# jai1215snu/ShiftedScaleQuantization

Hardware: AMD Instinct MI355X
Metric: Gelem/s shifted-scale q/dq + recon iters/s, ResNet-18 W2A4; top-1 vs ref (higher is better)
Workload: dtype f32; 1 GPU; resnet18 W2A4 bias_cal+bias_ch_quant, 1024 calib samples: A4 per-tensor q/dq of act [1024,64,56,56] + W2 per-channel q/dq of all 21 conv/fc weights (8-bit stem/head); parallelism=dp1

## Files before the change

include/ssq.h:

```cpp
#ifndef SSQ_H_
#define SSQ_H_

#include <stddef.h>
#include <stdint.h>

#ifdef __cplusplus
extern "C" {
#endif

#define SSQ_OK 0
#define SSQ_E_ARG (-1)
#define SSQ_E_WS (-2)

typedef void* ssq_stream_t;

const char* ssq_last_error(void);
int ssq_version(void);
int ssq_set_variant(int variant);

int ssq_fq_fwd(const float* x, float* y, void* codes_or_null, const float* delta,
               const float* zp, int64_t n, int64_t inner, int64_t nch, float scale,
               int qmin, int qmax, ssq_stream_t stream);
int ssq_fq_round_fwd(const float* x, float* y, void* codes_or_null, const float* delta,
                     const float* zp, int64_t n, int64_t inner, int64_t nch, float scale,
// ... 170 lines not shown
int ssq_epilogue_bwd(const float* g, const float* y, const float* bias, const float* gamma,
                     const float* phi, const float* res, int64_t N, int64_t C, int64_t hw,
                     int relu, const float* delta, const float* zp, int qmin, int qmax, float* gy,
                     float* gres, float* ggamma, float* gphi, float* gdelta, float* gzp, void* ws,
                     size_t ws_bytes, ssq_stream_t stream);
int ssq_epilogue_loss_bwd(const float* tgt_cache, const int64_t* idx, int64_t M, float p,
                          float* loss_out, const float* y, const float* bias, const float* gamma,
                          const float* phi, const float* res, const float* res_bias,
                          const float* res_gamma, const float* res_phi, int64_t N, int64_t C,
                          int64_t hw, int relu, const float* delta, const float* zp, int qmin,
                          int qmax, float* gy, float* gres, float* ggamma, float* gphi,
                          float* gres_gamma, float* gres_phi, float* gdelta, float* gzp,
                          void* ws, size_t ws_bytes, ssq_stream_t stream);
int ssq_epilogue_fwd_rows(const float* y, const int64_t* y_rows, const float* bias,
                          const float* gamma, const float* phi, const float* res,
                          const int64_t* res_rows, float* out, float* yq, int64_t n, int64_t hw,
                          int64_t C, int relu, const float* delta, const float* zp, int qmin,
                          int qmax, const int64_t* stage_src, int64_t* stage_dst,
                          int64_t stage_n, ssq_stream_t stream);
int ssq_epilogue_bwd_rows(const float* g, const float* y, const int64_t* y_rows,
                          const float* bias, const float* gamma, const float* phi,
                          const float* res, const int64_t* res_rows, int64_t N, int64_t C,
                          int64_t hw, int relu, const float* delta, const float* zp, int qmin,
                          int qmax, float* gy, float* gres, float* ggamma, float* gphi,
                          float* gdelta, float* gzp, void* ws, size_t ws_bytes,
                          ssq_stream_t stream);
int ssq_epilogue_loss_bwd_rows(const float* tgt_cache, const int64_t* idx, int64_t M, float p,
                               float* loss_out, const float* y, const int64_t* y_rows,
                               const float* bias, const float* gamma, const float* phi,
                               const float* res, const int64_t* res_rows,
                               const float* res_bias, const float* res_gamma,
                               const float* res_phi, int64_t N, int64_t C, int64_t hw, int relu,
                               const float* delta, const float* zp, int qmin, int qmax,
                               float* gy, float* gres, float* ggamma, float* gphi,
                               float* gres_gamma, float* gres_phi, float* gdelta, float* gzp,
                               void* ws, size_t ws_bytes, ssq_stream_t stream);

int ssq_adam(int nseg, float* const* p, const float* const* g, float* const* m,
             float* const* v, const int64_t* n, float one_minus_beta1, float beta2,
             float one_minus_beta2, float eps, const float* hyper, float neg_step_size,
             float bias_correction2_sqrt, ssq_stream_t stream);
int ssq_adam_arm(int nseg, float* const* p, float* const* m, float* const* v, const int64_t* n,
                 float one_minus_beta1, float beta2, float one_minus_beta2, float eps,
                 const float* hyper, ssq_stream_t stream);
int ssq_adam_take(ssq_stream_t stream);

int ssq_set_deferred_finalize(int on);
int ssq_flush_finalize(ssq_stream_t stream);

int ssq_set_deferred_prep_fwd(int on);
int ssq_flush_prep_fwd(ssq_stream_t stream);

int ssq_conv_wgrad_set_form(int form);
int ssq_conv_wgrad_kind(int64_t Nb, int64_t C, int64_t H, int64_t W, int64_t Co, int64_t R,
                        int64_t S, int64_t stride, int64_t pad, int64_t groups);
size_t ssq_conv_wgrad_workspace_size(int64_t Nb, int64_t C, int64_t H, int64_t W, int64_t Co,
                                     int64_t R, int64_t S, int64_t stride, int64_t pad,
                                     int64_t groups);
int ssq_conv_wgrad(const float* x, const float* dy, int64_t Nb, int64_t C, int64_t H, int64_t W,
                   int64_t Co, int64_t R, int64_t S, int64_t stride, int64_t pad, int64_t groups,
                   float* dw, void* ws, size_t ws_bytes, ssq_stream_t stream);
int ssq_wgrad_gemm_operands(const float* x, const float* dy, int64_t Nb, int64_t C, int64_t H,
                            int64_t W, int64_t Co, int64_t R, int64_t S, int64_t stride,
                            int64_t pad, float* col, float* dy2, ssq_stream_t stream);
int ssq_gemm_col_epilogue(const float* y, const float* bias, const float* gamma,
                          const float* phi, int relu, const float* delta, const float* zp,
                          int qmin, int qmax, int64_t Nb, int64_t C, int64_t H, int64_t W,
                          int64_t R, int64_t S, int64_t stride, int64_t pad, float* col,
                          ssq_stream_t stream);

int ssq_dwconv_supported(int64_t Nb, int64_t C, int64_t H, int64_t W, int64_t R, int64_t S,
                         int64_t stride, int64_t pad);
int ssq_dwconv_fwd(const float* x, const float* w, float* y, int64_t Nb, int64_t C, int64_t H,
                   int64_t W, int64_t R, int64_t S, int64_t stride, int64_t pad,
                   ssq_stream_t stream);
int ssq_dwconv_bwd_data(const float* dy, const float* w, float* dx, int64_t Nb, int64_t C,
                        int64_t H, int64_t W, int64_t R, int64_t S, int64_t stride, int64_t pad,
                        ssq_stream_t stream);

int ssq_pack_bits(int n_bits);
size_t ssq_pack_bytes(int64_t n, int n_bits);
int ssq_pack_encode(const float* What, const float* zp, const float* d1, int d1_per_ci,
                    const float* d2, int64_t Co, int64_t Ci, int64_t K, int n_bits, int qmin,
                    int qmax, void* packed, uint32_t* mismatch, ssq_stream_t stream);
int ssq_pack_decode(const void* packed, const float* zp, const float* d1, int d1_per_ci,
                    const float* d2, int64_t Co, int64_t Ci, int64_t K, int n_bits, int qmin,
                    float* What, ssq_stream_t stream);

int ssq_stream_copy(const float* src, float* dst, int64_t n, ssq_stream_t stream);
int ssq_stream_probe(const float* src, float* dst, int64_t n, int kind, ssq_stream_t stream);

#ifdef __cplusplus
}
#endif
#endif
```

shiftedscalequantization_amd/_capi.py:

```python
import ctypes as C
import os

import torch

_HERE = os.path.dirname(os.path.abspath(__file__))
LIB_PATH = os.environ.get("SSQ_LIB", os.path.join(_HERE, "libssq.so"))

_p = C.c_void_p
_i64 = C.c_int64
_i = C.c_int
_f = C.c_float
_sz = C.c_size_t

SIGNATURES = {
    "ssq_last_error": (C.c_char_p, []),
    "ssq_version": (_i, []),
    "ssq_set_variant": (_i, [_i]),
    "ssq_fq_fwd": (_i, [_p, _p, _p, _p, _p, _i64, _i64, _i64, _f, _i, _i, _p]),
    "ssq_fq_round_fwd": (_i, [_p, _p, _p, _p, _p, _i64, _i64, _i64, _f, _i, _i, _p]),
    "ssq_fq_fwd_multi": (_i, [_i, _p, _p, _p, _p, _p, _p, _p, _p, _p, _p]),
    "ssq_fq_bwd_workspace_size": (_sz, [_i64, _i64, _i64]),
    "ssq_fq_bwd": (_i, [_p, _p, _p, _p, _i64, _i64, _i64, _i, _i, _p, _p, _p, _p, _sz, _p]),
    "ssq_fq_round_bwd": (_i, [_p, _p, _p, _p, _i64, _i64, _i64, _i, _i, _p, _p, _p, _sz, _p]),
    "ssq_fq_relu_bwd": (_i, [_p, _p, _p, _p, _i64, _i, _i, _p, _p, _p, _p, _sz, _p]),
# ... 22 lines not shown
                              _f, _f, _p, _p, _p, _p, _p, _sz, _p]),
    "ssq_shift_reg": (_i, [_p, _i, _i64, _i, _f, _f, _p, _p, _p]),
    "ssq_lhs_fwd": (_i, [_p, _p, _p, _p, _p, _i, _i64, _i64, _i64, _i, _i, _i, _i, _p, _p]),
    "ssq_lhs_bwd": (_i, [_p, _p, _p, _p, _p, _p, _i, _i64, _i64, _i64, _i, _i, _i, _p, _p, _sz,
                         _p]),
    "ssq_adaround_fwd": (_i, [_p, _p, _p, _i, _p, _f, _i64, _i64, _i64, _i, _i, _i, _p, _p, _p]),
    "ssq_adaround_bwd": (_i, [_p, _p, _p, _p, _i, _p, _f, _i64, _i64, _i64, _i, _i, _f, _f, _p,
                              _p, _p]),
    "ssq_adaround_fwd_multi": (_i, [_i, _p, _p, _p, _p, _p, _p, _p, _p, _p, _i, _p, _p, _p, _p]),
    "ssq_adaround_bwd_multi": (_i, [_i, _p, _p, _p, _p, _p, _p, _p, _p, _p, _p, _p, _p, _f, _f,
                                    _p, _p, _p]),
    "ssq_round_reg_workspace_size": (_sz, [_i64]),
    "ssq_round_reg": (_i, [_p, _i64, _f, _f, _p, _p, _p, _sz, _p]),
    "ssq_inpscale_search": (_i, [_p, _p, _p, _i64, _i64, _i, _i, _f, _p, _p]),
    "ssq_inpscale_fwd": (_i, [_p, _p, _p, _p, _i64, _i64, _i, _p, _p]),
    "ssq_lp_loss_workspace_size": (_sz, [_i64]),
    "ssq_lp_loss": (_i, [_p, _p, _i64, _i64, _f, _p, _p, _p, _i, _p, _sz, _p]),
    "ssq_lp_loss_rows": (_i, [_p, _p, _p, _i64, _i64, _i64, _f, _p, _p, _p, _i, _p, _sz, _p]),
    "ssq_gather_rows2": (_i, [_p, _p, _i64, _p, _p, _i64, _p, _i64, _p]),
    "ssq_gemm_col_epilogue": (_i, [_p, _p, _p, _p, _i, _p, _p, _i, _i] + [_i64] * 8 + [_p, _p]),
    "ssq_fc_recon_workspace_size": (_sz, [_i64, _i64, _i64]),
    "ssq_fc_recon_iter": (_i, [_p, _p, _p, _i64, _p, _p, _p, _p, _p, _i, _i, _p, _i64, _i64, _f, _f,
                               _f, _f, _p, _p, _p, _p, _p, _p, _sz, _p]),
    "ssq_gather_rows2_staged": (_i, [_p, _p, _i64, _p, _p, _i64, _p, _i64, _p, _i64, _p]),
    "ssq_bias_act": (_i, [_p, _p, _p, _p, _i64, _i64, _i64, _i, _p]),
    "ssq_relu_bwd": (_i, [_p, _p, _p, _i64, _p]),
    "ssq_relu6_bwd": (_i, [_p, _p, _p, _i64, _p]),
    "ssq_bias_act_fq": (_i, [_p, _p, _p, _p, _p, _i64, _i64, _i64, _i, _p, _p, _i, _i, _p]),
    "ssq_epilogue_fwd": (_i, [_p, _p, _p, _p, _p, _p, _p, _i64, _i64, _i64, _i, _p, _p, _i, _i,
                              _p]),
    "ssq_epilogue_bwd_workspace_size": (_sz, [_i64]),
    "ssq_epilogue_bwd": (_i, [_p, _p, _p, _p, _p, _p, _i64, _i64, _i64, _i, _p, _p, _i, _i, _p,
                              _p, _p, _p, _p, _p, _p, _sz, _p]),
    "ssq_epilogue_loss_bwd": (_i, [_p, _p, _i64, _f, _p, _p, _p, _p, _p, _p, _p, _p, _p, _i64,
                                   _i64, _i64, _i, _p, _p, _i, _i, _p, _p, _p, _p, _p, _p, _p,
                                   _p, _p, _sz, _p]),
    "ssq_epilogue_fwd_rows": (_i, [_p, _p, _p, _p, _p, _p, _p, _p, _p, _i64, _i64, _i64, _i, _p,
                                   _p, _i, _i, _p, _p, _i64, _p]),
    "ssq_epilogue_bwd_rows": (_i, [_p, _p, _p, _p, _p, _p, _p, _p, _i64, _i64, _i64, _i, _p, _p,
                                   _i, _i, _p, _p, _p, _p, _p, _p, _p, _sz, _p]),
    "ssq_epilogue_loss_bwd_rows": (_i, [_p, _p, _i64, _f, _p, _p, _p, _p, _p, _p, _p, _p, _p, _p,
                                        _p, _i64, _i64, _i64, _i, _p, _p, _i, _i, _p, _p, _p, _p,
                                        _p, _p, _p, _p, _p, _sz, _p]),
    "ssq_adam": (_i, [_i, _p, _p, _p, _p, _p, _f, _f, _f, _f, _p, _f, _f, _p]),
    "ssq_adam_arm": (_i, [_i, _p, _p, _p, _p, _f, _f, _f, _f, _p, _p]),
    "ssq_adam_take": (_i, [_p]),
    "ssq_set_deferred_finalize": (_i, [_i]),
    "ssq_flush_finalize": (_i, [_p]),
    "ssq_set_deferred_prep_fwd": (_i, [_i]),
    "ssq_set_deferred_fq_multi": (_i, [_i]),
    "ssq_flush_fq_multi": (_i, [_p]),
    "ssq_flush_prep_fwd": (_i, [_p]),
    "ssq_conv_wgrad_set_form": (_i, [_i]),
    "ssq_conv_wgrad_kind": (_i, [_i64] * 10),
    "ssq_conv_wgrad_workspace_size": (_sz, [_i64] * 10),
    "ssq_conv_wgrad": (_i, [_p, _p] + [_i64] * 10 + [_p, _p, _sz, _p]),
    "ssq_wgrad_gemm_operands": (_i, [_p, _p] + [_i64] * 9 + [_p, _p, _p]),
    "ssq_maxpool2d_fwd": (_i, [_p, _p] + [_i64] * 7 + [_p]),
    "ssq_dwconv_supported": (_i, [_i64] * 8),
    "ssq_dwconv_fwd": (_i, [_p, _p, _p] + [_i64] * 8 + [_p]),
    "ssq_dwconv_bwd_data": (_i, [_p, _p, _p] + [_i64] * 8 + [_p]),
    "ssq_pack_bits": (_i, [_i]),
    "ssq_pack_bytes": (_sz, [_i64, _i]),
    "ssq_pack_encode": (_i, [_p, _p, _p, _i, _p, _i64, _i64, _i64, _i, _i, _i, _p, _p, _p]),
    "ssq_pack_decode": (_i, [_p, _p, _p, _i, _p, _i64, _i64, _i64, _i, _i, _p, _p]),
    "ssq_stream_copy": (_i, [_p, _p, _i64, _p]),
    "ssq_stream_probe": (_i, [_p, _p, _i64, _i, _p]),
}

_lib = None


class SSQError(RuntimeError):
    pass


def load():
    global _lib
    if _lib is not None:
        return _lib
    if not os.path.exists(LIB_PATH):
        raise SSQError(f"libssq.so not found at {LIB_PATH}; build it with "
                       "`python -m shiftedscalequantization_amd.build` (hipcc, gfx950)")
    lib = C.CDLL(LIB_PATH)
    for name, (res, args) in SIGNATURES.items():
        fn = getattr(lib, name)
        fn.restype = res
        fn.argtypes = args
    _lib = lib
    return lib


CALL_HOOK = None


def call(name, *args):
    lib = load()
    if CALL_HOOK is not None:
        CALL_HOOK(name, args)
    rc = getattr(lib, name)(*args)
    if rc != 0:
        msg = lib.ssq_last_error().decode(errors="replace")
        raise SSQError(f"{name} failed (rc={rc}): {msg}")


def query(name, *args):
# ... 95 lines not shown
```

shiftedscalequantization_amd/csrc/conv_wgrad.hip:

```cpp
#include <stdlib.h>

#include <algorithm>
#include <type_traits>

#include "ssq_common.h"

namespace ssq {

typedef float f32x16 __attribute__((ext_vector_type(16)));

constexpr int kUnr = 2;

struct WgradGeo {
  int Nb, C, H, W, Co, OH, OW, R, S, st, pad, G, Cig, Cog;
  int Ncol;
  int WM;
  int Pq;
  int lda;
  int chunks_per_n;
  int nchunks;
  int cps;
  int nsplit;
  int in_rows;
  int ci_span;
// ... 668 lines not shown
    const char* v = getenv("SSQ_K17_MAXLDS");
    return (int64_t)(v && *v ? atoll(v) : 160 * 1024);
  }();
  double best = 1e300;
  for (int wm : {1, 2, 4}) {
    for (int pq : {128, 64}) {
      const int TM = 64 * wm, TN = 256 / wm;
      const int64_t span = std::min<int64_t>(g.Cig, (TN - 1) / RS + 2);
      const int64_t orows = (pq - 1 + OW - 1) / OW + 1;
      const int64_t in_rows = (orows - 1) * st + R;
      const int64_t xtile = span * in_rows * Wp;
      if ((int64_t)wgrad_lds(wm, pq, xtile) > max_lds) continue;
      const int64_t cpn = (OH * OW + pq - 1) / pq;
      const int64_t tiles = ((g.Cog + TM - 1) / TM) * ((g.Ncol + TN - 1) / TN);
      const double dma = (double)(std::min<int64_t>(TM, g.Cog) * ((pq + 63) / 64) +
                                  span * in_rows * ((W + 63) / 64)) / 4.0;
      const double cost = (double)tiles * Nb * (2.0 * OH * OW + cpn * (40.0 + dma));
      if (cost < best) {
        best = cost;
        g.WM = wm;
        g.Pq = pq;
        g.ci_span = (int)span;
        g.in_rows = (int)in_rows;
        g.xtile = (int)xtile;
      }
    }
  }
  SSQ_REQUIRE(best < 1e300, SSQ_E_ARG, "ssq_conv_wgrad: input rows too wide for the LDS tile");
  const int TM = 64 * g.WM, TN = 256 / g.WM;
  g.lda = g.Pq + 1;
  g.chunks_per_n = (int)((OH * OW + g.Pq - 1) / g.Pq);
  g.nchunks = g.Nb * g.chunks_per_n;
  g.m_tiles = (g.Cog + TM - 1) / TM;
  g.n_tiles = (g.Ncol + TN - 1) / TN;
  const int64_t tiles = (int64_t)g.n_tiles * g.m_tiles * g.G;
  int nsplit = (int)std::max<int64_t>(1, std::min<int64_t>(g.nchunks / 2, (512 + tiles - 1) / tiles));
  g.cps = (g.nchunks + nsplit - 1) / nsplit;
  g.nsplit = (g.nchunks + g.cps - 1) / g.cps;
  *lds_bytes = wgrad_lds(g.WM, g.Pq, g.xtile);
  return SSQ_OK;
}

constexpr int kBandMaxNI = 20;
__device__ float g_band_zero_page[4 * 64];

struct BandGeo {
  int C, H, W, Co, OW, OHW, Cig, Cog;
  int RB, Q, Qp, PA, IR, PXrow, PXci;
  int TMc, CBc;
  int bufsz;
  int d16;
  int ni_w;
  int bands_per_n, nchunks, cps, nsplit, m_tiles, n_tiles, remap;
  FastDiv dPA, dPXci, dPXrow;
};

template <int N>
using IntC = std::integral_constant<int, N>;

template <int WMX, int ST, int V, int NWV>
__global__ __launch_bounds__(64 * NWV, 1) void wgrad_band_stage1(const float* __restrict__ x,
                                                                 const float* __restrict__ dy,
                                                                 BandGeo g, float* __restrict__ part) {
  static_assert(NWV == 4 || NWV == 8, "4 or 8 waves");
  constexpr int WNX = 4 / WMX;
  constexpr int kSlots = kBandMaxNI * 4 / NWV;
  extern __shared__ float lds[];
  const int tid = threadIdx.x, lane = tid & 63;
  const int wave = __builtin_amdgcn_readfirstlane(tid >> 6);
  const int wt = wave & 3, role = wave >> 2;
  const int wm = wt / WNX, wn = wt - wm * WNX;
  int wg = blockIdx.x;
  const int tiles = g.m_tiles * g.n_tiles;
  if (g.remap) {
    const int per = (int)gridDim.x >> 3;
    wg = (wg & 7) * per + (wg >> 3);
  }
  const int split = wg / tiles, tile = wg - split * tiles;
  const int mt = tile / g.n_tiles, nt = tile - mt * g.n_tiles;
  const int co0 = mt * g.TMc, ci0 = nt * g.CBc;
  const int c_begin = split * g.cps, c_end = min(c_begin + g.cps, g.nchunks);
  const int abytes = g.TMc * g.PA;
  const int n16 = g.d16 ? min(kSlots, (g.bufsz / 256 - wave + NWV - 1) / NWV) : 0;
  const int n4 = g.d16 ? 0 : (g.bufsz / 64 - wave + NWV - 1) / NWV;

  int soff[kSlots], meta[kSlots];
#pragma unroll
  for (int i = 0; i < kSlots; ++i) {
    soff[i] = 0;
    meta[i] = 0;
    if (i < n16) {
      const int o = (wave + NWV * i) * 256 + lane * 4;
      if (o < abytes) {
        const int row = (int)fdiv((uint32_t)o, g.dPA), col = o - row * g.PA;
        if (col < g.Q && co0 + row < g.Cog) {
          soff[i] = (co0 + row) * g.OHW + col;
          meta[i] = 1;
        }
      } else {
        const int o2 = o - abytes;
        const int cl = (int)fdiv((uint32_t)o2, g.dPXci), rem = o2 - cl * g.PXci;
        const int ir = (int)fdiv((uint32_t)rem, g.dPXrow), iw = rem - ir * g.PXrow - 4;
        if (cl < g.CBc && ci0 + cl < g.Cig && ir < g.IR && iw >= 0 && iw < g.W) {
          soff[i] = ((ci0 + cl) * g.H + ir) * g.W + iw;
          meta[i] = 2 | (ir << 2);
        }
      }
    }
  }
  struct Band {
    const float* ab;
    const float* xb;
    int ih0;
  };
  auto band_of = [&](int c) {
    const int n = c / g.bands_per_n;
    const int oh0 = (c - n * g.bands_per_n) * g.RB;
    const int ih0 = oh0 * ST - 1;
    return Band{dy + (int64_t)n * g.Co * g.OHW + oh0 * g.OW,
                x + (int64_t)n * g.C * g.H * g.W + (int64_t)ih0 * g.W, ih0};
  };
  auto stage16 = [&](const Band& bd, int b) {
    const float* zero = g_band_zero_page + lane * 4;
    float* dst = lds + b * g.bufsz + wave * 256;
#pragma unroll
    for (int i = 0; i < kSlots; ++i) {
      if (i < n16) {
        const int kind = meta[i] & 3;
        const unsigned ih = (unsigned)(bd.ih0 + (meta[i] >> 2));
        const bool ok = (kind == 1) | ((kind == 2) & (ih < (unsigned)g.H));
        const uint64_t pa = (uint64_t)(bd.ab + soff[i]), px = (uint64_t)(bd.xb + soff[i]);
        const uint64_t p = ok ? (kind == 1 ? pa : px) : (uint64_t)zero;
        __builtin_amdgcn_global_load_lds((const void*)p, (void*)(dst + i * NWV * 256), 16, 0, 0);
      }
    }
  };
  const int HW = g.H * g.W;
  auto stage4 = [&](const Band& bd, int b, int i0, int i1) {
    const float* zero = g_band_zero_page + lane;
    float* dst = lds + b * g.bufsz + wave * 64;
    for (int i = i0; i < i1; ++i) {
      const int o = (wave + NWV * i) * 64 + lane;
      const float* src = zero;
      if ((wave + NWV * i) * 64 < abytes) {
        const int row = (int)fdiv((uint32_t)o, g.dPA), col = o - row * g.PA;
        if (col < g.Q && co0 + row < g.Cog) src = bd.ab + (co0 + row) * g.OHW + col;
      } else {
        const int o2 = o - abytes;
        const int cl = (int)fdiv((uint32_t)o2, g.dPXci), rem = o2 - cl * g.PXci;
        const int ir = (int)fdiv((uint32_t)rem, g.dPXrow), iw = rem - ir * g.PXrow - 4;
        const unsigned ih = (unsigned)(bd.ih0 + ir);
        if (cl < g.CBc && ci0 + cl < g.Cig && ir < g.IR && iw >= 0 && iw < g.W &&
            ih < (unsigned)g.H)
          src = bd.xb + (ci0 + cl) * HW + ir * g.W + iw;
      }
      __builtin_amdgcn_global_load_lds((const void*)src, (void*)(dst + i * NWV * 64), 4, 0, 0);
    }
  };

  typedef float f32x4v __attribute__((ext_vector_type(4)));
  typedef float f32x2v __attribute__((ext_vector_type(2)));
  const int h = lane >> 5, l32 = lane & 31;
  const int arow = (wm * 32 + l32) * g.PA;
  const int xrow = abytes + (wn * 32 + l32) * g.PXci;
  const int q0 = h * (g.Qp >> 1);
  const int ngroups = g.Qp / (2 * V);
  const int last_row = (g.Q - 1) / g.OW, last_col = (g.Q - 1) - last_row * g.OW;
  constexpr int NW = (V - 1) * ST + 3;
  const int per_step = (n4 + max(1, ngroups / 2) - 1) / max(1, ngroups / 2);
  if (c_begin < c_end) {
    const Band bd = band_of(c_begin);
    if (g.d16) stage16(bd, 0);
    else stage4(bd, 0, 0, n4);
  }

  auto body = [&](auto t0c, auto t1c) {
    constexpr int T0 = decltype(t0c)::value, T1 = decltype(t1c)::value, NT = T1 - T0;
    constexpr int R0 = T0 / 3, NR = (T1 - 1) / 3 - R0 + 1;
    f32x16 acc[NT];
#pragma unroll
    for (int t = 0; t < NT; ++t) acc[t] = f32x16{0};
    auto fetch = [&](const float* L, int q, int orow, int ow, float (&a)[V],
                     float (&w)[NR][NW]) {
      if constexpr (V == 4) {
        const f32x4v av = *(const f32x4v*)(L + arow + q);
        a[0] = av.x; a[1] = av.y; a[2] = av.z; a[3] = av.w;
      } else if constexpr (V == 2) {
        const f32x2v av = *(const f32x2v*)(L + arow + q);
        a[0] = av.x; a[1] = av.y;
      } else {
        a[0] = L[arow + q];
      }
      int xr_row = orow, xr_col = ow;
      if (q >= g.Q) {
        xr_row = last_row;
        xr_col = last_col - (V - 1);
      }
      const float* xr0 = L + xrow + (xr_row * ST + R0) * g.PXrow + xr_col * ST + 3;
#pragma unroll
      for (int r = 0; r < NR; ++r) {
        const float* xr = xr0 + r * g.PXrow;
        if constexpr (V == 4) {
          w[r][0] = xr[0];
          const f32x4v t1 = *(const f32x4v*)(xr + 1);
          w[r][1] = t1.x; w[r][2] = t1.y; w[r][3] = t1.z; w[r][4] = t1.w;
          if constexpr (ST == 1) {
            w[r][5] = xr[5];
          } else {
            const f32x4v t2 = *(const f32x4v*)(xr + 5);
            w[r][5] = t2.x; w[r][6] = t2.y; w[r][7] = t2.z; w[r][8] = t2.w;
          }
        } else {
#pragma unroll
          for (int j = 0; j < NW; ++j) w[r][j] = xr[j];
        }
      }
    };
    auto mfmas = [&](const float (&a)[V], const float (&w)[NR][NW]) {
#pragma unroll
      for (int r = 0; r < NR; ++r)
#pragma unroll
        for (int v = 0; v < V; ++v)
#pragma unroll
          for (int s = 0; s < 3; ++s) {
            const int tap = (R0 + r) * 3 + s;
            if (tap >= T0 && tap < T1)
              acc[tap - T0] = __builtin_amdgcn_mfma_f32_32x32x2f32(a[v], w[r][v * ST + s],
                                                                   acc[tap - T0], 0, 0, 0);
          }
    };
    auto interleave = [&]() {
      constexpr int NM = NT * V, ND = NM < 12 ? NM : 12;
#pragma unroll
      for (int k = 0; k < ND; ++k) {
        __builtin_amdgcn_sched_group_barrier(0x008, 1, 0);
        __builtin_amdgcn_sched_group_barrier(0x100, 1, 0);
      }
      __builtin_amdgcn_sched_group_barrier(0x008, NM - ND, 0);
    };
    for (int c = c_begin; c < c_end; ++c) {
      const int b = (c - c_begin) & 1;
      asm volatile("s_waitcnt vmcnt(0)" ::: "memory");
      __syncthreads();
      const bool more = c + 1 < c_end;
      const Band nb = band_of(more ? c + 1 : c);
      if (more && g.d16) stage16(nb, b ^ 1);
      const float* L = lds + b * g.bufsz;
      int q = q0, orow = q0 / g.OW, ow = q0 - orow * g.OW;
      auto advance = [&]() {
        q += V;
        ow += V;
        if (ow == g.OW) {
          ow = 0;
          ++orow;
        }
      };
      auto stage_slice = [&](int gi) {
        if (more && !g.d16) {
          const int i0 = gi * per_step;
          if (i0 < n4) stage4(nb, b ^ 1, i0, min(i0 + per_step, n4));
        }
      };
      float a0[V], w0[NR][NW], a1[V], w1[NR][NW];
      fetch(L, q, orow, ow, a0, w0);
      const int npairs = ngroups >> 1;
      for (int gp = 0; gp < npairs; ++gp) {
        stage_slice(2 * gp);
        advance();
        fetch(L, q, orow, ow, a1, w1);
        mfmas(a0, w0);
        interleave();
        stage_slice(2 * gp + 1);
        advance();
        fetch(L, q, orow, ow, a0, w0);
        mfmas(a1, w1);
        interleave();
      }
      if (ngroups & 1) {
        stage_slice(ngroups - 1);
        mfmas(a0, w0);
      }
    }
    const int co_w = co0 + wm * 32, ci = ci0 + wn * 32 + l32;
    if (ci < g.Cig) {
#pragma unroll
      for (int t = 0; t < NT; ++t) {
        float* dst = part + ((int64_t)split * 9 + T0 + t) * g.Cog * g.Cig;
#pragma unroll
        for (int i = 0; i < 16; ++i) {
          const int co = co_w + (i & 3) + 8 * (i >> 2) + 4 * h;
          if (co < g.Cog) dst[(int64_t)co * g.Cig + ci] = acc[t][i];
        }
      }
    }
  };
  if constexpr (NWV == 4) {
    body(IntC<0>{}, IntC<9>{});
  } else {
    if (role == 0) body(IntC<0>{}, IntC<5>{});
    else body(IntC<5>{}, IntC<9>{});
  }
}

static int g_wgrad_form = 0;
static int band_waves() {
  static const int w = [] {
    const char* e = getenv("SSQ_BAND_WAVES");
    return e && *e && atoi(e) == 4 ? 4 : 8;
  }();
  return g_wgrad_form == 4 ? 4 : w;
}

static int band_plan(int64_t Nb, int64_t C, int64_t H, int64_t W, int64_t Co, int64_t R,
                     int64_t S, int64_t st, int64_t pad, int64_t G, BandGeo& g, int* wmx,
                     int* vpx) {
  if (G != 1 || R != 3 || S != 3 || pad != 1 || (st != 1 && st != 2)) return 0;
  const int64_t OH = (H + 2 - 3) / st + 1, OW = (W + 2 - 3) / st + 1;
  if (OH < 1 || OW < 1 || Co % 32 || C % 32) return 0;
  if (Nb * C * H * W >= (1ll << 31) || Nb * Co * OH * OW >= (1ll << 31)) return 0;
  g.C = (int)C; g.H = (int)H; g.W = (int)W; g.Co = (int)Co; g.OW = (int)OW;
  g.OHW = (int)(OH * OW); g.Cig = (int)C; g.Cog = (int)Co;
  const int V = OW % 4 == 0 ? 4 : (OW % 2 == 0 ? 2 : 1);
  auto odd4 = [](int v) { v = (v + 3) / 4 * 4; return (v / 4) % 2 ? v : v + 4; };
  const int64_t budget = 160 * 1024 / 2 / 4;
  bool found = false;
  double best = 1e300;
  for (int wm : {2, 4}) {
    const int TMc = 32 * wm, CBc = 32 * (4 / wm);
    if (wm == 4 && Co < 128) continue;
    for (int rb = (int)std::min<int64_t>(OH, 8); rb >= 1; --rb) {
      if (OH % rb) continue;
      const int Q = rb * (int)OW, Qp = (Q + 2 * V - 1) / (2 * V) * (2 * V);
      const int IR = (rb - 1) * (int)st + 3;
      const bool d16 = W % 4 == 0 && g.OHW % 4 == 0 && Q % 4 == 0 && Qp == Q;
      const int need = (int)((OW - 1) * st) + 6;
      const int PXrow = d16 ? (int)W + 8 : (std::max<int>(need, (int)W + 4) + 3) / 4 * 4;
      const int PA = odd4(Qp + 1), PXci = odd4(IR * PXrow);
      const int64_t buf = ((int64_t)TMc * PA + (int64_t)CBc * PXci + 1023) / 1024 * 1024;
      if (buf > budget) continue;
      const int ni = d16 ? (int)(buf / 1024) : (int)(buf / 256);
      if (d16 && ni > kBandMaxNI) continue;
      const double cost = (288.0 * Qp + 1500.0 + (d16 ? 40.0 : 10.0) * ni) / Q;
      if (cost >= best) continue;
      best = cost;
      g.RB = rb; g.Q = Q; g.Qp = Qp; g.PA = PA; g.IR = IR; g.PXrow = PXrow; g.PXci = PXci;
      g.TMc = TMc; g.CBc = CBc; g.bufsz = (int)buf; g.d16 = d16 ? 1 : 0; g.ni_w = ni;
      *wmx = wm;
      *vpx = V;
      found = true;
    }
  }
  if (!found) return 0;
  g.dPA = make_fastdiv((uint32_t)g.PA);
  g.dPXci = make_fastdiv((uint32_t)g.PXci);
  g.dPXrow = make_fastdiv((uint32_t)g.PXrow);
  g.m_tiles = (g.Cog + g.TMc - 1) / g.TMc;
  g.n_tiles = (g.Cig + g.CBc - 1) / g.CBc;
  g.bands_per_n = (int)(OH / g.RB);
  g.nchunks = (int)Nb * g.bands_per_n;
  const int tiles = g.m_tiles * g.n_tiles;
  int ns = std::max(1, std::min(g.nchunks, (256 + tiles - 1) / tiles));
  g.cps = (g.nchunks + ns - 1) / ns;
  g.nsplit = (g.nchunks + g.cps - 1) / g.cps;
  g.remap = ((int64_t)g.nsplit * tiles) % 8 == 0;
  return 1;
}

static bool use_band(int64_t Nb, int64_t C, int64_t H, int64_t W, int64_t Co, int64_t R,
                     int64_t S, int64_t st, int64_t pad, int64_t G, BandGeo& g, int* wmx,
                     int* vpx) {
  if (g_wgrad_form != 0 && g_wgrad_form != 3 && g_wgrad_form != 4) return false;
  return band_plan(Nb, C, H, W, Co, R, S, st, pad, G, g, wmx, vpx) != 0;
}
static bool use_i2c(int64_t R, int64_t S, int64_t Co, int64_t G) {
  if (g_wgrad_form != 0) return g_wgrad_form == 2;
  return R * S > 1 && G == 1 && Co >= 128;
}

}

using namespace ssq;

extern "C" int ssq_conv_wgrad_set_form(int form) {
  const int old = g_wgrad_form;
  if (form >= 0 && form <= 4) g_wgrad_form = form;
  return old;
}

extern "C" int ssq_conv_wgrad_kind(int64_t Nb, int64_t C, int64_t H, int64_t W, int64_t Co,
                                   int64_t R, int64_t S, int64_t stride, int64_t pad,
                                   int64_t groups) {
  if (is_depthwise(C, Co, groups) && R * S <= 25 && Nb >= 1 && dw_lds_ok(H, W, pad)) return 5;
  BandGeo gb;
  int wmx, vpx;
  if (use_band(Nb, C, H, W, Co, R, S, stride, pad, groups, gb, &wmx, &vpx)) return gb.d16 ? 3 : 6;
  if (use_i2c(R, S, Co, groups)) {
    I2cGeo gi;
    return wgrad_i2c_plan(Nb, C, H, W, Co, R, S, stride, pad, groups, gi) ? 0 : 2;
  }
  if (R == 1 && S == 1 && pad == 0) {
    W1Geo g1;
    return wgrad_1x1_plan(Nb, C, H, W, Co, stride, groups, g1) ? 0 : 4;
  }
  WgradGeo g;
  size_t lds;
  return wgrad_plan(Nb, C, H, W, Co, R, S, stride, pad, groups, g, &lds) ? 0 : 1;
}

extern "C" size_t ssq_conv_wgrad_workspace_size(int64_t Nb, int64_t C, int64_t H, int64_t W,
                                                int64_t Co, int64_t R, int64_t S, int64_t stride,
                                                int64_t pad, int64_t groups) {
  if (is_depthwise(C, Co, groups) && R * S <= 25 && Nb >= 1 && dw_lds_ok(H, W, pad)) {
    int spl;
    const int ns = dw_splits(Nb, C, &spl);
    const int64_t OH = (H + 2 * pad - R) / stride + 1;
    int64_t nbands = 1;
    if (dw_stage(H, W, pad, spl) == 0 && OH >= 1) {
      const int bh = dw_band_rows(H, W, R, stride, pad, OH);
      nbands = (OH + bh - 1) / bh;
    }
    return (size_t)ns * (size_t)nbands * (size_t)C * (size_t)(R * S) * sizeof(float);
  }
  {
    BandGeo gb;
    int wmx, vpx;
    if (use_band(Nb, C, H, W, Co, R, S, stride, pad, groups, gb, &wmx, &vpx))
      return (size_t)gb.nsplit * 9 * (size_t)Co * (size_t)C * sizeof(float);
  }
  if (use_i2c(R, S, Co, groups)) {
    I2cGeo gi;
    int wm;
    if (wgrad_i2c_plan(Nb, C, H, W, Co, R, S, stride, pad, groups, gi)) return 0;
    wgrad_i2c_tiles(gi, &wm);
    return (size_t)gi.nsplit * (size_t)Co * (size_t)gi.Ncol * sizeof(float);
  }
  if (R == 1 && S == 1 && pad == 0) {
    W1Geo g1;
    if (wgrad_1x1_plan(Nb, C, H, W, Co, stride, groups, g1)) return 0;
    return (size_t)g1.nsplit * (size_t)Co * (size_t)g1.Cig * sizeof(float);
// ... 34 lines not shown
      else
        hipLaunchKernelGGL(wgrad_dw_small<25>, grid, dim3(256), lds, s, x, dy, (int)C, (int)H,
                           (int)W, (int)OH, (int)OW, (int)R, (int)S, (int)stride, (int)pad, spl,
                           nb, dWp, dP, dOHW, dOW, (float*)ws);
      const int64_t n = C * R * S;
      hipLaunchKernelGGL(wgrad_stage2, dim3((unsigned)std::min<int64_t>((n + 63) / 64, 4096)),
                         dim3(256), 0, s, (const float*)ws, ns, n, dw);
      return check_launch("ssq_conv_wgrad");
    }
    const int bh = dw_band_rows(H, W, R, stride, pad, OH);
    const int nbands = (int)((OH + bh - 1) / bh);
    SSQ_REQUIRE(ws_bytes >= need * (size_t)nbands, SSQ_E_WS, "ssq_conv_wgrad: workspace too small");
    const dim3 gridb((unsigned)C, (unsigned)(ns * nbands));
    const size_t lds = (size_t)(((int64_t)bh - 1) * stride + R) * (W + 2 * pad) * sizeof(float);
    static bool dw_attr = false;
    if (!dw_attr) {
      hipFuncSetAttribute((const void*)wgrad_dw_stage1<9>,
                          hipFuncAttributeMaxDynamicSharedMemorySize, 128 * 1024);
      hipFuncSetAttribute((const void*)wgrad_dw_stage1<25>,
                          hipFuncAttributeMaxDynamicSharedMemorySize, 128 * 1024);
      dw_attr = true;
    }
    if (R * S <= 9)
      hipLaunchKernelGGL(wgrad_dw_stage1<9>, gridb, dim3(256), lds, s, x, dy, (int)C, (int)H, (int)W,
                         (int)OH, (int)OW, (int)R, (int)S, (int)stride, (int)pad, spl, bh, nbands,
                         make_fastdiv((uint32_t)(W + 2 * pad)), (float*)ws);
    else
      hipLaunchKernelGGL(wgrad_dw_stage1<25>, gridb, dim3(256), lds, s, x, dy, (int)C, (int)H, (int)W,
                         (int)OH, (int)OW, (int)R, (int)S, (int)stride, (int)pad, spl, bh, nbands,
                         make_fastdiv((uint32_t)(W + 2 * pad)), (float*)ws);
    const int64_t n = C * R * S;
    hipLaunchKernelGGL(wgrad_stage2, dim3((unsigned)std::min<int64_t>((n + 63) / 64, 4096)),
                       dim3(256), 0, s, (const float*)ws, ns * nbands, n, dw);
    return check_launch("ssq_conv_wgrad");
  }
  {
    BandGeo gb;
    int wmx, vpx;
    if (use_band(Nb, C, H, W, Co, R, S, stride, pad, groups, gb, &wmx, &vpx)) {
      const size_t needb = (size_t)gb.nsplit * 9 * (size_t)Co * (size_t)C * sizeof(float);
      SSQ_REQUIRE(ws && ws_bytes >= needb, SSQ_E_WS, "ssq_conv_wgrad: workspace too small");
      typedef void (*BandK)(const float*, const float*, BandGeo, float*);
#define SSQ_BK(NWV)                                                                          \
  {{{wgrad_band_stage1<2, 1, 4, NWV>, wgrad_band_stage1<2, 1, 2, NWV>,                        \
     wgrad_band_stage1<2, 1, 1, NWV>},                                                        \
    {wgrad_band_stage1<2, 2, 4, NWV>, wgrad_band_stage1<2, 2, 2, NWV>,                        \
     wgrad_band_stage1<2, 2, 1, NWV>}},                                                       \
   {{wgrad_band_stage1<4, 1, 4, NWV>, wgrad_band_stage1<4, 1, 2, NWV>,                        \
     wgrad_band_stage1<4, 1, 1, NWV>},                                                        \
    {wgrad_band_stage1<4, 2, 4, NWV>, wgrad_band_stage1<4, 2, 2, NWV>,                        \
     wgrad_band_stage1<4, 2, 1, NWV>}}}
      static const BandK kernels[2][2][2][3] = {SSQ_BK(4), SSQ_BK(8)};
#undef SSQ_BK
      static bool band_attr = false;
      if (!band_attr) {
        for (auto& a0 : kernels)
          for (auto& a : a0)
            for (auto& b : a)
              for (BandK k : b)
                hipFuncSetAttribute((const void*)k, hipFuncAttributeMaxDynamicSharedMemorySize,
                                    160 * 1024);
        band_attr = true;
      }
      const int w8 = band_waves() == 8;
      const BandK kb = kernels[w8][wmx == 4][stride == 2][vpx == 4 ? 0 : (vpx == 2 ? 1 : 2)];
      const dim3 gridb((unsigned)(gb.nsplit * gb.m_tiles * gb.n_tiles));
      const size_t ldsb = 2 * (size_t)gb.bufsz * sizeof(float);
      hipLaunchKernelGGL(kb, gridb, dim3(w8 ? 512 : 256), ldsb, s, x, dy, gb, (float*)ws);
      const int64_t inner = Co * C, nb = 9 * inner;
      hipLaunchKernelGGL(wgrad_stage2, dim3((unsigned)std::min<int64_t>((nb + 63) / 64, 4096)),
                         dim3(256), 0, s, (const float*)ws, gb.nsplit, nb, dw, inner, 9);
      return check_launch("ssq_conv_wgrad");
    }
  }
  if (use_i2c(R, S, Co, groups)) {
    I2cGeo gi;
    int wm;
    const int rci = wgrad_i2c_plan(Nb, C, H, W, Co, R, S, stride, pad, groups, gi);
    if (rci) return rci;
    wgrad_i2c_tiles(gi, &wm);
    const size_t needi = (size_t)gi.nsplit * (size_t)Co * (size_t)gi.Ncol * sizeof(float);
    SSQ_REQUIRE(ws && ws_bytes >= needi, SSQ_E_WS, "ssq_conv_wgrad: workspace too small");
    const dim3 gridi(gi.n_tiles, gi.m_tiles * gi.G, gi.nsplit);
    (void)wm;
    hipLaunchKernelGGL(wgrad_i2c_stage1<2>, gridi, dim3(256), 0, s, x, dy, gi, (float*)ws);
    const int64_t ni = (int64_t)Co * gi.Ncol;
    hipLaunchKernelGGL(wgrad_stage2, dim3((unsigned)std::min<int64_t>((ni + 63) / 64, 4096)),
                       dim3(256), 0, s, (const float*)ws, gi.nsplit, ni, dw);
    return check_launch("ssq_conv_wgrad");
  }
  if (R == 1 && S == 1 && pad == 0) {
    W1Geo g1;
    const int rc1 = wgrad_1x1_plan(Nb, C, H, W, Co, stride, groups, g1);
    if (rc1) return rc1;
    const size_t need1 = (size_t)g1.nsplit * (size_t)Co * (size_t)g1.Cig * sizeof(float);
    SSQ_REQUIRE(ws && ws_bytes >= need1, SSQ_E_WS, "ssq_conv_wgrad: workspace too small");
    const dim3 grid1(g1.n_tiles, g1.m_tiles * g1.G, g1.nsplit);
    hipLaunchKernelGGL(wgrad_1x1_stage1<2>, grid1, dim3(256), 0, s, x, dy, g1, (float*)ws);
    const int64_t n1 = (int64_t)Co * g1.Cig;
    hipLaunchKernelGGL(wgrad_stage2, dim3((unsigned)std::min<int64_t>((n1 + 63) / 64, 4096)),
                       dim3(256), 0, s, (const float*)ws, g1.nsplit, n1, dw);
    return check_launch("ssq_conv_wgrad");
  }
  WgradGeo g;
  size_t lds;
  int rc = wgrad_plan(Nb, C, H, W, Co, R, S, stride, pad, groups, g, &lds);
  if (rc) return rc;
  const size_t need = (size_t)g.nsplit * (size_t)Co * (size_t)g.Ncol * sizeof(float);
  SSQ_REQUIRE(ws && ws_bytes >= need, SSQ_E_WS, "ssq_conv_wgrad: workspace too small");
  static bool lds_attr = false;
  if (!lds_attr) {
    hipFuncSetAttribute((const void*)wgrad_stage1<1>, hipFuncAttributeMaxDynamicSharedMemorySize,
                        160 * 1024);
    hipFuncSetAttribute((const void*)wgrad_stage1<2>, hipFuncAttributeMaxDynamicSharedMemorySize,
                        160 * 1024);
    hipFuncSetAttribute((const void*)wgrad_stage1<4>, hipFuncAttributeMaxDynamicSharedMemorySize,
                        160 * 1024);
    lds_attr = true;
  }
  const dim3 grid(g.n_tiles, g.m_tiles * g.G, g.nsplit);
// ... 171 lines not shown
```

shiftedscalequantization_amd/kernels.py:

```python
import ctypes as C
import os

import torch

from . import _capi as A
from ._capi import call, fptr, query, stream_of, workspace


def qrange(n_bits, sym):
    n = 2 ** n_bits
    return (-(n // 2), n // 2 - 1) if sym else (0, n - 1)


def geometry(w):
    if w.dim() == 4:
        return int(w.shape[0]), int(w.shape[1]), int(w.shape[2] * w.shape[3]), 0
    if w.dim() == 2:
        return int(w.shape[0]), int(w.shape[1]), 1, 1
    raise ValueError(f"weight must be 2-D (Linear) or 4-D (Conv2d), got {tuple(w.shape)}")


def _codes_buf(x, want):
    return torch.empty(x.shape, dtype=torch.uint8, device=x.device) if want else None

# ... 1411 lines not shown
    packed = torch.empty(max(nbytes, 1), dtype=torch.uint8, device=w.device)[:nbytes]
    bad = torch.zeros(1, dtype=torch.int32, device=w.device)
    call("ssq_pack_encode", wp, zpp, ap, int(per_ci), bp, Co, Ci, Kk, n_bits, qmin, qmax,
         _vp(packed), _vp(bad), stream_of(w))
    return packed, int(bad.item())


def pack_decode(packed, shape, zp, d1, per_ci, d2, n_bits, qmin):
    if packed.device.type != "cuda" or packed.dtype != torch.uint8:
        raise A.SSQError("pack_decode: packed codes must be a uint8 tensor on the HIP device")
    out = torch.empty(shape, dtype=torch.float32, device=packed.device)
    Co, Ci, Kk, _ = geometry(out)
    if packed.numel() < query("ssq_pack_bytes", out.numel(), n_bits):
        raise A.SSQError("pack_decode: packed buffer too small for the shape")
    packed = packed.contiguous()
    z, zpp = fptr(zp.reshape(-1), "zero_point")
    a, ap = fptr(d1.reshape(-1), "scale")
    b, bp = fptr(d2.reshape(-1), "col_scale") if d2 is not None else (None, None)
    call("ssq_pack_decode", _vp(packed), zpp, ap, int(per_ci), bp, Co, Ci, Kk, n_bits, qmin,
         _vp(out), stream_of(out))
    return out


def conv_wgrad_supported(x, weight, stride, padding, dilation, groups):
    if x.dim() != 4 or weight.dim() != 4 or not x.is_cuda or x.dtype != torch.float32:
        return False
    st = stride if isinstance(stride, int) else stride[0]
    pad = padding if isinstance(padding, int) else padding[0]
    if not isinstance(stride, int) and len(set(stride)) != 1:
        return False
    if not isinstance(padding, int) and (isinstance(padding, str) or len(set(padding)) != 1):
        return False
    if (dilation if isinstance(dilation, int) else max(dilation)) != 1:
        return False
    Nb, C, H, W = (int(v) for v in x.shape)
    Co, _, R, S = (int(v) for v in weight.shape)
    return query("ssq_conv_wgrad_workspace_size", Nb, C, H, W, Co, R, S, int(st), int(pad),
                 int(groups)) > 0


def wgrad_kind(x_shape, w_shape, stride, padding, groups):
    st = stride if isinstance(stride, int) else stride[0]
    pad = padding if isinstance(padding, int) else padding[0]
    Nb, C, H, W = (int(v) for v in x_shape)
    Co, _, R, S = (int(v) for v in w_shape)
    return int(query("ssq_conv_wgrad_kind", Nb, C, H, W, Co, R, S, int(st), int(pad),
                     int(groups)))


def set_wgrad_form(form):
    return int(query("ssq_conv_wgrad_set_form", int(form)))


def conv_wgrad(x, dy, w_shape, stride, padding, groups):
    st = stride if isinstance(stride, int) else stride[0]
    pad = padding if isinstance(padding, int) else padding[0]
    x, xp = fptr(x.detach(), "x")
    dy, dp = fptr(dy.detach(), "dy")
    Nb, C, H, W = (int(v) for v in x.shape)
    Co, _, R, S = (int(v) for v in w_shape)
    dims = (Nb, C, H, W, Co, R, S, int(st), int(pad), int(groups))
    ws, wsn = workspace(query("ssq_conv_wgrad_workspace_size", *dims), x.device)
    dw = torch.empty(tuple(w_shape), dtype=torch.float32, device=x.device)
    call("ssq_conv_wgrad", xp, dp, *dims, _vp(dw), ws, wsn, stream_of(x))
    return dw


def _gemm_geo(x_shape, w_shape, stride, padding):
    st = stride if isinstance(stride, int) else stride[0]
    pad = padding if isinstance(padding, int) else padding[0]
    Nb, C_, H, W = (int(v) for v in x_shape)
    Co, _, R, S = (int(v) for v in w_shape)
    OH, OW = (H + 2 * pad - R) // st + 1, (W + 2 * pad - S) // st + 1
    return Nb, C_, H, W, Co, R, S, int(st), int(pad), OH, OW


def gemm_operands(x, dy, w_shape, stride, padding, want_col=True, want_dy2=True):
    shape = x.shape if x is not None else None
    Nb, C_, H, W, Co, R, S, st, pad, OH, OW = _gemm_geo(shape, w_shape, stride, padding)
    NP = Nb * OH * OW
    dev_ = (x if x is not None else dy).device
    col = torch.empty(NP, C_ * R * S, dtype=torch.float32, device=dev_) if want_col else None
    dy2 = torch.empty(Co, NP, dtype=torch.float32, device=dev_) if want_dy2 else None
    xt, xp = fptr(x.detach(), "x") if want_col else (None, None)
    dt, dp = fptr(dy.detach(), "dy") if want_dy2 else (None, None)
    call("ssq_wgrad_gemm_operands", xp, dp, Nb, C_, H, W, Co, R, S, st, pad, _vp(col), _vp(dy2),
         stream_of(col if want_col else dy2))
    return col, dy2


def conv_wgrad_gemm(x, dy, w_shape, stride, padding, col=None):
    c2, dy2 = gemm_operands(x if col is None else x, dy, w_shape, stride, padding,
                            want_col=col is None, want_dy2=True)
    col = c2 if col is None else col
    return torch.matmul(dy2, col).view(tuple(w_shape))


def conv_fwd_gemm(x, weight, stride, padding):
    Nb, C_, H, W, Co, R, S, st, pad, OH, OW = _gemm_geo(x.shape, weight.shape, stride, padding)
    col, _ = gemm_operands(x, None, weight.shape, stride, padding, want_col=True, want_dy2=False)
    y = torch.matmul(weight.detach().reshape(Co, C_ * R * S),
                     col.view(Nb, OH * OW, C_ * R * S).transpose(1, 2))
    return y.view(Nb, Co, OH, OW), col


def dwconv_supported(x, weight, stride, padding, dilation, groups):
# ... 342 lines not shown
```

Measured before the change: 709.6 Gelem/s.

## Add row-ring LDS reuse of input rows across bands in stride-1 wgrad band kernel

Adds a ring-buffer variant of the band wgrad stage-1 kernel for stride-1, 16-byte rows with 8 waves. Input rows that overlap between consecutive bands of the same image stay in LDS, and only the new RB rows are staged per band, so halo rows are not reloaded. The ring is refilled at image boundaries with an extra sync. It is enabled by default when LDS and slot limits fit, with a new form 5 to turn it off and a plan query API. Risks are extra index arithmetic and a sync stall at image boundaries.

```diff
diff --git a/include/ssq.h b/include/ssq.h
--- a/include/ssq.h
+++ b/include/ssq.h
@@ -246,6 +246,8 @@
 int ssq_flush_prep_fwd(ssq_stream_t stream);
 
 int ssq_conv_wgrad_set_form(int form);
+int ssq_conv_wgrad_band_plan(int64_t Nb, int64_t C, int64_t H, int64_t W, int64_t Co,
+                             int64_t stride, int* plan);
 int ssq_conv_wgrad_kind(int64_t Nb, int64_t C, int64_t H, int64_t W, int64_t Co, int64_t R,
                         int64_t S, int64_t stride, int64_t pad, int64_t groups);
 size_t ssq_conv_wgrad_workspace_size(int64_t Nb, int64_t C, int64_t H, int64_t W, int64_t Co,
diff --git a/shiftedscalequantization_amd/_capi.py b/shiftedscalequantization_amd/_capi.py
--- a/shiftedscalequantization_amd/_capi.py
+++ b/shiftedscalequantization_amd/_capi.py
@@ -98,6 +98,7 @@
     "ssq_flush_fq_multi": (_i, [_p]),
     "ssq_flush_prep_fwd": (_i, [_p]),
     "ssq_conv_wgrad_set_form": (_i, [_i]),
+    "ssq_conv_wgrad_band_plan": (_i, [_i64] * 6 + [_p]),
     "ssq_conv_wgrad_kind": (_i, [_i64] * 10),
     "ssq_conv_wgrad_workspace_size": (_sz, [_i64] * 10),
     "ssq_conv_wgrad": (_i, [_p, _p] + [_i64] * 10 + [_p, _p, _sz, _p]),
diff --git a/shiftedscalequantization_amd/csrc/conv_wgrad.hip b/shiftedscalequantization_amd/csrc/conv_wgrad.hip
--- a/shiftedscalequantization_amd/csrc/conv_wgrad.hip
+++ b/shiftedscalequantization_amd/csrc/conv_wgrad.hip
@@ -744,17 +744,19 @@
   int d16;
   int ni_w;
   int bands_per_n, nchunks, cps, nsplit, m_tiles, n_tiles, remap;
-  FastDiv dPA, dPXci, dPXrow;
+  int ring, NS, RP, slotsz, SP, nA;
+  FastDiv dPA, dPXci, dPXrow, dRP, dSP;
 };
 
 template <int N>
 using IntC = std::integral_constant<int, N>;
 
-template <int WMX, int ST, int V, int NWV>
+template <int WMX, int ST, int V, int NWV, int RING = 0>
 __global__ __launch_bounds__(64 * NWV, 1) void wgrad_band_stage1(const float* __restrict__ x,
                                                                  const float* __restrict__ dy,
                                                                  BandGeo g, float* __restrict__ part) {
   static_assert(NWV == 4 || NWV == 8, "4 or 8 waves");
+  static_assert(!RING || (ST == 1 && V == 4), "the row ring is for stride 1, 16-B rows");
   constexpr int WNX = 4 / WMX;
   constexpr int kSlots = kBandMaxNI * 4 / NWV;
   extern __shared__ float lds[];
@@ -773,15 +775,34 @@
   const int co0 = mt * g.TMc, ci0 = nt * g.CBc;
   const int c_begin = split * g.cps, c_end = min(c_begin + g.cps, g.nchunks);
   const int abytes = g.TMc * g.PA;
-  const int n16 = g.d16 ? min(kSlots, (g.bufsz / 256 - wave + NWV - 1) / NWV) : 0;
+  const int n16 = g.d16 && !RING ? min(kSlots, (g.bufsz / 256 - wave + NWV - 1) / NWV) : 0;
   const int n4 = g.d16 ? 0 : (g.bufsz / 64 - wave + NWV - 1) / NWV;
+  const int ja0 = NWV - 1 - wave;
+  const int nAw = RING ? min(kSlots, (g.nA - ja0 + NWV - 1) / NWV) : 0;
+  const int nXw = RING ? min(kSlots, (g.RB * g.SP - wave + NWV - 1) / NWV) : 0;
+  float* const ring = lds + 2 * abytes;
 
   int soff[kSlots], meta[kSlots];
 #pragma unroll
   for (int i = 0; i < kSlots; ++i) {
     soff[i] = 0;
     meta[i] = 0;
-    if (i < n16) {
+    if constexpr (RING) {
+      soff[i] = -1;
+      meta[i] = -1;
+      if (i < nAw) {
+        const int o = (ja0 + NWV * i) * 256 + lane * 4;
+        const int row = (int)fdiv((uint32_t)o, g.dPA), col = o - row * g.PA;
+        if (col < g.Q && co0 + row < g.Cog) soff[i] = (co0 + row) * g.OHW + col;
+      }
+      if (i < nXw) {
+        const int p = wave + NWV * i, j = p - (int)fdiv((uint32_t)p, g.dSP) * g.SP;
+        const int o = j * 256 + lane * 4;
+        const int cl = (int)fdiv((uint32_t)o, g.dRP), iw = o - cl * g.RP - 4;
+        if (cl < g.CBc && ci0 + cl < g.Cig && iw >= 0 && iw < g.W)
+          meta[i] = (ci0 + cl) * g.H * g.W + iw;
+      }
+    } else if (i < n16) {
       const int o = (wave + NWV * i) * 256 + lane * 4;
       if (o < abytes) {
         const int row = (int)fdiv((uint32_t)o, g.dPA), col = o - row * g.PA;
@@ -824,6 +845,50 @@
         const uint64_t pa = (uint64_t)(bd.ab + soff[i]), px = (uint64_t)(bd.xb + soff[i]);
         const uint64_t p = ok ? (kind == 1 ? pa : px) : (uint64_t)zero;
         __builtin_amdgcn_global_load_lds((const void*)p, (void*)(dst + i * NWV * 256), 16, 0, 0);
+      }
+    }
+  };
+  auto ring_slot = [&](int s) { return s >= g.NS ? s - g.NS : s; };
+  auto stage_a = [&](int n, int cb, int b) {
+    const float* zero = g_band_zero_page + lane * 4;
+    const float* ab = dy + (int64_t)n * g.Co * g.OHW + cb * g.RB * g.OW;
+    float* dst = lds + b * abytes + ja0 * 256;
+#pragma unroll
+    for (int i = 0; i < kSlots; ++i) {
+      if (i < nAw) {
+        const uint64_t p = soff[i] >= 0 ? (uint64_t)(ab + soff[i]) : (uint64_t)zero;
+        __builtin_amdgcn_global_load_lds((const void*)p, (void*)(dst + i * NWV * 256), 16, 0, 0);
+      }
+    }
+  };
+  auto stage_new = [&](int n, int cb, int bs) {
+    const float* zero = g_band_zero_page + lane * 4;
+    const float* xs = x + (int64_t)n * g.C * g.H * g.W;
+#pragma unroll
+    for (int i = 0; i < kSlots; ++i) {
+      if (i < nXw) {
+        const int p = wave + NWV * i, k = (int)fdiv((uint32_t)p, g.dSP), j = p - k * g.SP;
+        const int ih = cb * g.RB + 1 + k;
+        const bool ok = (meta[i] >= 0) & ((unsigned)ih < (unsigned)g.H);
+        const uint64_t src = ok ? (uint64_t)(xs + (ih * g.W + meta[i])) : (uint64_t)zero;
+        float* dst = ring + ring_slot(bs + 2 + k) * g.slotsz + j * 256;
+        __builtin_amdgcn_global_load_lds((const void*)src, (void*)dst, 16, 0, 0);
+      }
+    }
+  };
+  auto stage_fill = [&](int n, int cb) {
+    const float* zero = g_band_zero_page + lane * 4;
+    const float* xs = x + (int64_t)n * g.C * g.H * g.W;
+    for (int t = 0; t < g.IR; ++t) {
+      const int ih = cb * g.RB - 1 + t;
+      for (int j = wave; j < g.SP; j += NWV) {
+        const int o = j * 256 + lane * 4;
+        const int cl = (int)fdiv((uint32_t)o, g.dRP), iw = o - cl * g.RP - 4;
+        const bool ok = cl < g.CBc && ci0 + cl < g.Cig && iw >= 0 && iw < g.W &&
+                        (unsigned)ih < (unsigned)g.H;
+        const float* src = ok ? xs + (((ci0 + cl) * g.H + ih) * g.W + iw) : zero;
+        __builtin_amdgcn_global_load_lds((const void*)src,
+                                         (void*)(ring + t * g.slotsz + j * 256), 16, 0, 0);
       }
     }
   };
@@ -855,15 +920,23 @@
   const int h = lane >> 5, l32 = lane & 31;
   const int arow = (wm * 32 + l32) * g.PA;
   const int xrow = abytes + (wn * 32 + l32) * g.PXci;
+  const int xlane = (wn * 32 + l32) * g.RP;
   const int q0 = h * (g.Qp >> 1);
   const int ngroups = g.Qp / (2 * V);
   const int last_row = (g.Q - 1) / g.OW, last_col = (g.Q - 1) - last_row * g.OW;
   constexpr int NW = (V - 1) * ST + 3;
   const int per_step = (n4 + max(1, ngroups / 2) - 1) / max(1, ngroups / 2);
+  const int n_begin = RING ? c_begin / g.bands_per_n : 0;
+  const int cb_begin = c_begin - n_begin * g.bands_per_n;
   if (c_begin < c_end) {
-    const Band bd = band_of(c_begin);
-    if (g.d16) stage16(bd, 0);
-    else stage4(bd, 0, 0, n4);
+    if constexpr (RING) {
+      stage_a(n_begin, cb_begin, 0);
+      stage_fill(n_begin, cb_begin);
+    } else {
+      const Band bd = band_of(c_begin);
+      if (g.d16) stage16(bd, 0);
+      else stage4(bd, 0, 0, n4);
+    }
   }
 
   auto body = [&](auto t0c, auto t1c) {
@@ -872,6 +945,7 @@
     f32x16 acc[NT];
 #pragma unroll
     for (int t = 0; t < NT; ++t) acc[t] = f32x16{0};
+    int bs = 0;
     auto fetch = [&](const float* L, int q, int orow, int ow, float (&a)[V],
                      float (&w)[NR][NW]) {
       if constexpr (V == 4) {
@@ -888,10 +962,12 @@
         xr_row = last_row;
         xr_col = last_col - (V - 1);
       }
-      const float* xr0 = L + xrow + (xr_row * ST + R0) * g.PXrow + xr_col * ST + 3;
+      const float* xr0 = RING ? ring + xlane + xr_col + 3
+                              : L + xrow + (xr_row * ST + R0) * g.PXrow + xr_col * ST + 3;
 #pragma unroll
       for (int r = 0; r < NR; ++r) {
-        const float* xr = xr0 + r * g.PXrow;
+        const float* xr =
+            RING ? xr0 + ring_slot(bs + xr_row + R0 + r) * g.slotsz : xr0 + r * g.PXrow;
         if constexpr (V == 4) {
           w[r][0] = xr[0];
           const f32x4v t1 = *(const f32x4v*)(xr + 1);
@@ -930,14 +1006,35 @@
       }
       __builtin_amdgcn_sched_group_barrier(0x008, NM - ND, 0);
     };
+    int rn = n_begin, rcb = cb_begin;
     for (int c = c_begin; c < c_end; ++c) {
       const int b = (c - c_begin) & 1;
       asm volatile("s_waitcnt vmcnt(0)" ::: "memory");
       __syncthreads();
       const bool more = c + 1 < c_end;
-      const Band nb = band_of(more ? c + 1 : c);
-      if (more && g.d16) stage16(nb, b ^ 1);
-      const float* L = lds + b * g.bufsz;
+      const Band nb = RING ? Band{dy, x, 0} : band_of(more ? c + 1 : c);
+      if constexpr (RING) {
+        if (c != c_begin && rcb == 0) {
+          bs = 0;
+          stage_fill(rn, 0);
+          asm volatile("s_waitcnt vmcnt(0)" ::: "memory");
+          __syncthreads();
+        }
+        int n1 = rn, cb1 = rcb + 1;
+        if (cb1 == g.bands_per_n) {
+          ++n1;
+          cb1 = 0;
+        }
+        if (more) {
+          stage_a(n1, cb1, b ^ 1);
+          if (cb1) stage_new(n1, cb1, ring_slot(bs + g.RB));
+        }
+        rn = n1;
+        rcb = cb1;
+      } else {
+        if (more && g.d16) stage16(nb, b ^ 1);
+      }
+      const float* L = lds + b * (RING ? abytes : g.bufsz);
       int q = q0, orow = q0 / g.OW, ow = q0 - orow * g.OW;
       auto advance = [&]() {
         q += V;
@@ -948,7 +1045,7 @@
         }
       };
       auto stage_slice = [&](int gi) {
-        if (more && !g.d16) {
+        if (!RING && more && !g.d16) {
           const int i0 = gi * per_step;
           if (i0 < n4) stage4(nb, b ^ 1, i0, min(i0 + per_step, n4));
         }
@@ -972,6 +1069,7 @@
         stage_slice(ngroups - 1);
         mfmas(a0, w0);
       }
+      if constexpr (RING) bs = ring_slot(bs + g.RB);
     }
     const int co_w = co0 + wm * 32, ci = ci0 + wn * 32 + l32;
     if (ci < g.Cig) {
@@ -1007,6 +1105,7 @@
                      int64_t S, int64_t st, int64_t pad, int64_t G, BandGeo& g, int* wmx,
                      int* vpx) {
   if (G != 1 || R != 3 || S != 3 || pad != 1 || (st != 1 && st != 2)) return 0;
+  const bool ring_form = g_wgrad_form != 5 && band_waves() == 8;
   const int64_t OH = (H + 2 - 3) / st + 1, OW = (W + 2 - 3) / st + 1;
   if (OH < 1 || OW < 1 || Co % 32 || C % 32) return 0;
   if (Nb * C * H * W >= (1ll << 31) || Nb * Co * OH * OW >= (1ll << 31)) return 0;
@@ -1055,13 +1154,28 @@
   g.cps = (g.nchunks + ns - 1) / ns;
   g.nsplit = (g.nchunks + g.cps - 1) / g.cps;
   g.remap = ((int64_t)g.nsplit * tiles) % 8 == 0;
+  g.ring = 0;
+  g.RP = odd4(g.PXrow);
+  g.slotsz = (g.CBc * g.RP + 255) / 256 * 256;
+  g.SP = g.slotsz / 256;
+  g.NS = g.IR + g.RB;
+  g.nA = g.TMc * g.PA / 256;
+  g.dRP = make_fastdiv((uint32_t)g.RP);
+  g.dSP = make_fastdiv((uint32_t)g.SP);
+  if (g.d16 && st == 1 && ring_form) {
+    const int64_t lds_floats = 2 * (int64_t)g.TMc * g.PA + (int64_t)g.NS * g.slotsz;
+    const int per_wave = kBandMaxNI / 2;
+    if (lds_floats * 4 <= 160 * 1024 && (g.nA + 7) / 8 <= per_wave &&
+        (g.RB * g.SP + 7) / 8 <= per_wave)
+      g.ring = 1;
+  }
   return 1;
 }
 
 static bool use_band(int64_t Nb, int64_t C, int64_t H, int64_t W, int64_t Co, int64_t R,
                      int64_t S, int64_t st, int64_t pad, int64_t G, BandGeo& g, int* wmx,
                      int* vpx) {
-  if (g_wgrad_form != 0 && g_wgrad_form != 3 && g_wgrad_form != 4) return false;
+  if (g_wgrad_form != 0 && g_wgrad_form < 3) return false;
   return band_plan(Nb, C, H, W, Co, R, S, st, pad, G, g, wmx, vpx) != 0;
 }
 static bool use_i2c(int64_t R, int64_t S, int64_t Co, int64_t G) {
@@ -1075,8 +1189,18 @@
 
 extern "C" int ssq_conv_wgrad_set_form(int form) {
   const int old = g_wgrad_form;
-  if (form >= 0 && form <= 4) g_wgrad_form = form;
+  if (form >= 0 && form <= 5) g_wgrad_form = form;
   return old;
+}
+
+extern "C" int ssq_conv_wgrad_band_plan(int64_t Nb, int64_t C, int64_t H, int64_t W, int64_t Co,
+                                        int64_t stride, int* plan) {
+  BandGeo gb;
+  int wmx, vpx;
+  if (!plan || !use_band(Nb, C, H, W, Co, 3, 3, stride, 1, 1, gb, &wmx, &vpx)) return 0;
+  const int v[8] = {gb.TMc, gb.CBc, gb.RB, gb.cps, gb.nsplit, gb.bands_per_n, gb.ring, gb.NS};
+  for (int i = 0; i < 8; ++i) plan[i] = v[i];
+  return 1;
 }
 
 extern "C" int ssq_conv_wgrad_kind(int64_t Nb, int64_t C, int64_t H, int64_t W, int64_t Co,
@@ -1217,6 +1341,8 @@
      wgrad_band_stage1<4, 2, 1, NWV>}}}
       static const BandK kernels[2][2][2][3] = {SSQ_BK(4), SSQ_BK(8)};
 #undef SSQ_BK
+      static const BandK ring_kernels[2] = {wgrad_band_stage1<2, 1, 4, 8, 1>,
+                                            wgrad_band_stage1<4, 1, 4, 8, 1>};
       static bool band_attr = false;
       if (!band_attr) {
         for (auto& a0 : kernels)
@@ -1225,12 +1351,19 @@
               for (BandK k : b)
                 hipFuncSetAttribute((const void*)k, hipFuncAttributeMaxDynamicSharedMemorySize,
                                     160 * 1024);
+        for (BandK k : ring_kernels)
+          hipFuncSetAttribute((const void*)k, hipFuncAttributeMaxDynamicSharedMemorySize,
+                              160 * 1024);
         band_attr = true;
       }
       const int w8 = band_waves() == 8;
-      const BandK kb = kernels[w8][wmx == 4][stride == 2][vpx == 4 ? 0 : (vpx == 2 ? 1 : 2)];
+      SSQ_REQUIRE(!gb.ring || (w8 && stride == 1 && vpx == 4), SSQ_E_ARG,
+                  "ssq_conv_wgrad: band plan");
+      const BandK kb = gb.ring ? ring_kernels[wmx == 4]
+                               : kernels[w8][wmx == 4][stride == 2][vpx == 4 ? 0 : (vpx == 2 ? 1 : 2)];
       const dim3 gridb((unsigned)(gb.nsplit * gb.m_tiles * gb.n_tiles));
-      const size_t ldsb = 2 * (size_t)gb.bufsz * sizeof(float);
+      const size_t ldsb = (gb.ring ? 2 * (size_t)gb.TMc * gb.PA + (size_t)gb.NS * gb.slotsz
+                                   : 2 * (size_t)gb.bufsz) * sizeof(float);
       hipLaunchKernelGGL(kb, gridb, dim3(w8 ? 512 : 256), ldsb, s, x, dy, gb, (float*)ws);
       const int64_t inner = Co * C, nb = 9 * inner;
       hipLaunchKernelGGL(wgrad_stage2, dim3((unsigned)std::min<int64_t>((nb + 63) / 64, 4096)),
diff --git a/shiftedscalequantization_amd/kernels.py b/shiftedscalequantization_amd/kernels.py
--- a/shiftedscalequantization_amd/kernels.py
+++ b/shiftedscalequantization_amd/kernels.py
@@ -1487,6 +1487,17 @@
     return int(query("ssq_conv_wgrad_set_form", int(form)))
 
 
+def wgrad_band_plan(x_shape, co, stride):
+    import ctypes
+    Nb, C, H, W = (int(v) for v in x_shape)
+    plan = (ctypes.c_int * 8)()
+    if not query("ssq_conv_wgrad_band_plan", Nb, C, H, W, int(co), int(stride), plan):
+        return None
+    v = list(plan)
+    return {"tile": (v[0], v[1]), "rb": v[2], "cps": v[3], "nsplit": v[4], "bands_per_n": v[5],
+            "ring": v[6], "slots": v[7]}
+
+
 def conv_wgrad(x, dy, w_shape, stride, padding, groups):
     st = stride if isinstance(stride, int) else stride[0]
     pad = padding if isinstance(padding, int) else padding[0]
```

Result: no change. 713.5 Gelem/s (median of 3 runs) (+0.6%).
